# locuoco/coulomb_oscillators

Hardware: AMD Instinct MI355X
Metric: particle-steps/sec (+ Gpair-interactions/sec), N=1048576 FMM-3D kd-tree p=6, 1 GPU(s) (higher is better)
Workload: dtype f32; 1 GPU; FMM-3D kd-tree p=6, N=1048576 per GPU (one system of 1048576), leapfrog, Gaussian ball, tree rebuilt every 1 step(s); n_per_gpu=1048576, order=6, parallelism=single GPU, L=15, p2p_pairs=2017200, m2l_pairs=570291, build_mode=0, warm_builds=281, warm_misses=10, near_field=one-directional

## Files before the change

coulomb_oscillators_amd/csrc/k_fmm_kd.hip:

```cpp
#include "nbco_internal.hpp"
#include "k_p2p.hpp"
#include "kd_common.hpp"
#include "host_util.hpp"
#include <chrono>
#include <cmath>
#include <algorithm>
#include <vector>

namespace {

using kdc::wave_scan_add;
using kdc::wave_min_u32;

constexpr int sym_off(int n) { return n * (n + 1) * (n + 2) / 6; }
constexpr int tl_off(int n) { return n * n; }

struct TreeView
{
	float *center, *lbound, *rbound;
	float4 *csz;
	float *mpole, *local;
	int *mult, *index, *splitdim;
	int L, ntot;
};
// ... 50 lines not shown
	__host__ __device__ uint64_t operator()(unsigned cnt) const { return (uint64_t)cnt | ((uint64_t)((cnt + kP2PChunk - 1) / kP2PChunk) << 32); }
};
struct SplitRef
{
	int *s, *o;
	__host__ __device__ SplitRef &operator=(uint64_t v) { *s = (int)(uint32_t)v; *o = (int)(v >> 32); return *this; }
};
struct SplitIter
{
	using iterator_category = std::random_access_iterator_tag;
	using value_type = uint64_t;
	using difference_type = std::ptrdiff_t;
	using pointer = uint64_t *;
	using reference = SplitRef;
	int *s, *o;
	__host__ __device__ SplitRef operator*() const { return SplitRef{s, o}; }
	__host__ __device__ SplitRef operator[](difference_type i) const { return SplitRef{s + i, o + i}; }
	__host__ __device__ SplitIter operator+(difference_type i) const { return SplitIter{s + i, o + i}; }
	__host__ __device__ SplitIter operator-(difference_type i) const { return SplitIter{s - i, o - i}; }
	__host__ __device__ SplitIter &operator+=(difference_type i) { s += i; o += i; return *this; }
	__host__ __device__ SplitIter &operator++() { ++s; ++o; return *this; }
	__host__ __device__ difference_type operator-(const SplitIter &b) const { return s - b.s; }
};
static int build_directed_list(nbco_ctx *c, const int2 *pairs, const int2 *ranks, const int *pref_dev, long long capR, long long npairs_hint, int sub,
                               int self0, int nself, int ntargets, int shift, unsigned *cnt, int *start, uint64_t *keys_tmp, uint64_t *keys_out,
                               DevBuf &scan_tmp, const int *leaf_index = nullptr, const int *leaf_mult = nullptr, int2 *desc = nullptr,
                               int *chunk_off = nullptr, int4 *chunks = nullptr, const MutualLists *mutual = nullptr)
{
	hipStream_t st = c->stream;
	if (desc)
	{
		NBCO_TRY(exclusive_scan(c, scan_tmp, rocprim::make_transform_iterator((const unsigned *)cnt, PackCounts{}), SplitIter{start, chunk_off}, (uint64_t)0,
		                        (size_t)(ntargets + 1)));
	}
	else
		NBCO_TRY(exclusive_scan(c, scan_tmp, (int *)cnt, start, 0, (size_t)(ntargets + 1)));
	hipLaunchKernelGGL(list_fill_kernel, dim3(grid1d(npairs_hint + nself)), dim3(kBlock), 0, st, pairs, ranks, pref_dev, capR, sub, self0, nself, shift,
	                   (const int *)start, keys_tmp, (const int *)chunk_off, ntargets, leaf_index, leaf_mult,
	                   (desc && !mutual) ? chunks : (int4 *)nullptr, mutual ? 1 : 0);
	if (desc)
	{
		MutualLists mu;
		if (mutual) { mu = *mutual; mu.chunk = chunks; mu.chunk_off = chunk_off; mu.self0 = self0; mu.nself = nself; }
		const bool long_kernel = shift >= 11 && shift <= 16 && c->hint_np2p > 0 && 2 * c->hint_np2p > 48LL * (nself > 0 ? nself : ntargets);
		const int long_from = long_kernel ? 512 : 0;
		c->info.long_lists = long_kernel ? 1 : 0;
		hipLaunchKernelGGL(list_segsort_kernel<true>, dim3((ntargets + kBlock / 64 - 1) / (kBlock / 64)), dim3(kBlock), 0, st, (const int *)start, ntargets,
		                   keys_tmp, keys_out, shift, leaf_index, leaf_mult, desc, mu, long_from);
		if (long_kernel)
			hipLaunchKernelGGL(list_longsort_kernel, dim3(256), dim3(kLongBlock), 0, st, (const int *)start,
			                   ntargets, (const uint64_t *)keys_tmp, keys_out, shift, leaf_index, leaf_mult, desc, mu, long_from);
	}
	else
// ... 165 lines not shown
                                                           const unsigned char *__restrict__ have, int *__restrict__ host_word)
{
	const uint64_t mask = (1ull << shift) - 1;
	const int n = *total;
	int missing = 0;
	for (int i = blockIdx.x * kBlock + threadIdx.x; i < n; i += gridDim.x * kBlock)
	{
		const int id = (int)(keys[i] & mask);
		if (!have[id]) missing = id + 1;
	}
	if (missing) { *host_word = missing; __threadfence_system(); }
}
static int launch_let_guard(nbco_ctx *c, const uint64_t *keys, const int *total, int shift, const unsigned char *have, int word, long long hint)
{
	hipLaunchKernelGGL(let_guard_kernel, dim3(grid1d(hint, 2048)), dim3(kBlock), 0, c->stream, keys, total, shift, have,
	                   c->h_flags + kLetWord + 2 * (int)(c->dist.let_epoch & 1) + word);
	NBCO_HIP(hipGetLastError());
	return NBCO_OK;
}

struct KdCounts
{
	long long np2p = 0, nm2l = 0;
	int sel_overflow = 0, react_overflow = 0;
};

static int kd_list_room(nbco_ctx *c, int ntot, long long &capR, long long &cap)
{
	capR = 2 * (((long long)c->o.list_factor * c->list_growth * ntot + 4096 + kTravK - 1) / kTravK);
	cap = capR * kTravK;
	NBCO_TRY(c->reserve(c->frontier_a, sizeof(int2) * (size_t)cap));
	NBCO_TRY(c->reserve(c->frontier_b, sizeof(int2) * (size_t)cap));
	NBCO_TRY(c->reserve(c->p2p_list, sizeof(int2) * 2 * (size_t)cap));
	NBCO_TRY(c->reserve(c->m2l_list, sizeof(int2) * 2 * (size_t)cap));
	NBCO_TRY(c->reserve(c->counters, sizeof(int) * 128));
	c->list_cap = cap;
	return NBCO_OK;
}

static int kd_traverse(nbco_ctx *c, const TreeView &tv, long long n, const Dom dm)
{
	const int L = tv.L, ntot = tv.ntot, nleaf = 1 << L;
	const int self0 = dm.g << (L - dm.d), nself = 1 << (L - dm.d);
	hipStream_t st = c->stream;
	long long capR, cap;
	NBCO_TRY(kd_list_room(c, ntot, capR, cap));
	PhaseScope ph(c, NBCO_PH_TRAVERSE);
	AdmTab tab;
	for (int l = 0; l < 32; ++l)
	{
		long long lo = l <= L ? (n >> l) : 0;
		long long hi = l <= L ? ((n + (1LL << l) - 1) >> l) : 0;
		tab.lo[l] = (int)lo;
		const float e = 1.f / (float)(3 * c->o.fmm_order + 6);
		tab.Mlo[l] = lo > 0 ? std::pow((float)lo / (float)n, e) : 0.f;
		tab.Mhi[l] = hi > 0 ? std::pow((float)hi / (float)n, e) : 0.f;
	}
	int *ctr = c->counters.as<int>();
	int2 *fa = c->frontier_a.as<int2>(), *fb = c->frontier_b.as<int2>();
	const size_t np_ = (size_t)nleaf + 2, nm_ = (size_t)ntot + 2;
	NBCO_TRY(c->reserve(c->list_cnt, sizeof(unsigned) * 2 * (np_ + nm_)));
	unsigned *cnt_p2p = c->list_cnt.as<unsigned>(), *cnt_m2l = cnt_p2p + 2 * np_;
	NBCO_TRY(c->reserve(c->trav_ctr, sizeof(int) * 1024));
	static_assert(kTcInts <= 1024, "traversal counter block");
	int *tctr = c->trav_ctr.as<int>();
	NBCO_TRY(c->flags_begin());
	hipLaunchKernelGGL(traverse_init_kernel, dim3(grid1d((long long)(2 * (np_ + nm_)) / 8 + 1, 256)), dim3(kBlock), 0, st, fa, ctr, 104, tctr,
	                   c->list_cnt.as<unsigned>(), (long long)(2 * (np_ + nm_)), (long long)self0, (long long)(c->o.coll ? nself : 0));
	const int iters = L + NBCO_TRAV_EXTRA;
	for (int it = 0; it < iters; ++it)
	{
		hipLaunchKernelGGL(traverse_kernel, dim3(1024), dim3(kBlock), 0, st, tv, tab, (const int2 *)fa, fb, c->p2p_list.as<int2>(),
		                   c->m2l_list.as<int2>(), c->p2p_list.as<int2>() + cap, c->m2l_list.as<int2>() + cap, ctr, tctr, it, capR,
		                   c->o.tree_radius, c->o.m2l_first, cnt_p2p, cnt_m2l, dm);
		std::swap(fa, fb);
	}
	hipLaunchKernelGGL(traverse_finish_kernel, dim3(1), dim3(1024), 0, st, ctr, tctr, capR, c->list_cnt.as<unsigned>(), (long long)(2 * (np_ + nm_)),
	                   cnt_p2p + self0, c->o.coll ? nself : 0, c->h_flags, iters, ++c->flags_seq);
	NBCO_HIP(hipGetLastError());
	NBCO_HIP(hipEventRecord(c->ev_flags, st));
	return NBCO_OK;
}

static int kd_no_pre_far() { return NBCO_OK; }

template <class PreFar>
static int kd_fields(nbco_ctx *c, const TreeView &tv, const float4 *pos, long long n, int mlt_max, const Dom dm, long long own0, long long own_n,
                     const int *unsort, float *a, const float *param, KdCounts &out, PreFar pre_far, const LetHave *let = nullptr)
{
	const int P = c->o.fmm_order;
	const int L = tv.L, ntot = tv.ntot, nleaf = 1 << L, beg = kd_beg(L);
	const int offL = tl_off(P + 1);
	out = KdCounts{};
	const int self0 = dm.g << (L - dm.d), nself = 1 << (L - dm.d);
	long long capR, cap;
	NBCO_TRY(kd_list_room(c, ntot, capR, cap));
	const int *p2p_pref = c->trav_ctr.as<int>() + kTcP2PPref, *m2l_pref = c->trav_ctr.as<int>() + kTcM2LPref;
	const int shift = L + 1;
	const long long dp2p_cap = c->o.coll ? 2 * cap + nself : 0, dm2l_cap = 2 * cap;
	const long long np2p_hint = c->hint_np2p > 0 ? std::min(cap, c->hint_np2p + c->hint_np2p / 4 + 1024) : cap;
	const long long nm2l_hint = c->hint_nm2l > 0 ? std::min(cap, c->hint_nm2l + c->hint_nm2l / 4 + 1024) : cap;
	const long long dp2p_hint = 2 * np2p_hint + nself;
	const long long max_chunks = c->o.coll ? dp2p_cap / kP2PChunk + nself : 0, chunks_hint = dp2p_hint / kP2PChunk + nself;
	const int mutual_th = (c->o.coll && c->o.p2p_mutual) ? p2p_mutual_halves(mlt_max) : 0;
	const bool mutual = mutual_th > 0;
	c->info.p2p_halves = mutual_th;
	long long react_cap = 0;
	if (mutual)
	{
		if (c->hint_np2p <= 0)
		{
			NBCO_TRY(c->wait_flags());
			c->hint_np2p = c->h_flags[0];
			c->hint_nm2l = c->h_flags[1];
		}
		const long long pairs_room = std::min(cap, c->hint_np2p + c->hint_np2p / 4 + 1024);
		react_cap = 2 * pairs_room + nself;
		NBCO_TRY(c->reserve(c->p2p_react, sizeof(float4) * 32 * (size_t)mutual_th * (size_t)react_cap));
	}
	float4 *near = nullptr;
	auto enqueue_p2p = [&]() -> int {
		NBCO_TRY(c->reserve(c->part, sizeof(float4) * (size_t)max_chunks * (size_t)mlt_max));
		near = c->part.as<float4>();
		PhaseScope ph(c, NBCO_PH_P2P);
		const int4 *pc = c->p2p_chunks.as<int4>();
		const int *pt = c->p2p_chunk_off.as<int>() + nleaf;
		const int2 *pd = c->p2p_desc.as<int2>();
		if (mutual)
		{
			launch_p2p_mutual(c, mutual_th, pos, c->p2p_desc.as<int4>(), pc, pt, chunks_hint, mlt_max, near, c->p2p_react.as<float4>(), react_cap, n);
		}
		else if (mlt_max <= 8) launch_p2p<8>(c, pos, pd, pc, pt, chunks_hint, mlt_max, mlt_max, near, n);
		else if (mlt_max <= 16) launch_p2p<16>(c, pos, pd, pc, pt, chunks_hint, mlt_max, mlt_max, near, n);
		else if (mlt_max <= 32) launch_p2p<32>(c, pos, pd, pc, pt, chunks_hint, mlt_max, mlt_max, near, n);
		else launch_p2p<64>(c, pos, pd, pc, pt, chunks_hint, mlt_max, mlt_max, near, n);
		NBCO_HIP(hipGetLastError());
		static const char *dump_path = std::getenv("NBCO_P2P_DUMP");
		if (dump_path && !mutual) NBCO_TRY(p2p_dump(c, dump_path, pos, pd, pc, pt, c->p2p_start.as<int>() + nleaf, mlt_max, near, n));
		return NBCO_OK;
	};
	{
		NBCO_TRY(c->reserve(c->p2p_keys, sizeof(uint64_t) * (size_t)(dp2p_cap + 1)));
		NBCO_TRY(c->reserve(c->p2p_keys_alt, sizeof(uint64_t) * (size_t)(dp2p_cap + 1)));
		NBCO_TRY(c->reserve(c->m2l_keys, sizeof(uint64_t) * (size_t)(dm2l_cap + 1)));
		NBCO_TRY(c->reserve(c->m2l_keys_alt, sizeof(uint64_t) * (size_t)(dm2l_cap + 1)));
		NBCO_TRY(c->reserve(c->p2p_start, sizeof(int) * (size_t)(nleaf + 2)));
		NBCO_TRY(c->reserve(c->m2l_start, sizeof(int) * (size_t)(ntot + 2)));
		NBCO_TRY(c->fork_mark());
		if (c->o.coll)
		{
			PhaseScope ph(c, NBCO_PH_LISTS);
			unsigned *cp = c->list_cnt.as<unsigned>();
			NBCO_TRY(c->reserve(c->p2p_desc, (mutual ? sizeof(int4) : sizeof(int2)) * (size_t)(dp2p_cap + 1)));
			MutualLists mu;
			if (mutual)
			{
				NBCO_TRY(c->reserve(c->p2p_sec, sizeof(int2) * (size_t)(nleaf + 2)));
				mu.desc4 = c->p2p_desc.as<int4>();
				mu.sec_range = c->p2p_sec.as<int2>();
			}
			NBCO_TRY(c->reserve(c->p2p_chunk_off, sizeof(int) * (size_t)(nleaf + 2)));
			NBCO_TRY(c->reserve(c->p2p_chunks, sizeof(int4) * (size_t)max_chunks));
			NBCO_TRY(build_directed_list(c, c->p2p_list.as<int2>(), c->p2p_list.as<int2>() + cap, p2p_pref, capR, np2p_hint, beg, self0, nself, nleaf, shift, cp,
			                             c->p2p_start.as<int>(), c->p2p_keys.as<uint64_t>(), c->p2p_keys_alt.as<uint64_t>(), c->sort_tmp,
			                             tv.index + beg, tv.mult + beg, c->p2p_desc.as<int2>(), c->p2p_chunk_off.as<int>(), c->p2p_chunks.as<int4>(),
			                             mutual ? &mu : nullptr));
			if (mutual) launch_p2p_link(c, c->p2p_desc.as<int4>(), c->p2p_keys_alt.as<uint64_t>(), c->p2p_start.as<int>(), c->p2p_start.as<int>() + nleaf, shift, dp2p_hint);
			if (let) NBCO_TRY(launch_let_guard(c, c->p2p_keys_alt.as<uint64_t>(), c->p2p_start.as<int>() + nleaf, shift, let->leaf, 1, dp2p_hint));
			c->pc_mult = tv.mult + beg; c->pc_shift = shift; c->pc_total = c->p2p_start.as<int>() + nleaf;
		}
		if (c->o.coll) NBCO_TRY(enqueue_p2p());
		const int f64 = c->o.far_fp64 ? 1 : 0;
		NBCO_HIP(hipMemsetAsync(tv.local, 0, (f64 ? sizeof(double) : sizeof(float)) * (size_t)ntot * offL, c->aux));
		NBCO_TRY(c->fork_wait());
		{
			StreamScope on_aux(c, c->aux);
			NBCO_TRY(pre_far());
			unsigned *cm = c->list_cnt.as<unsigned>() + 2 * ((size_t)nleaf + 2);
			NBCO_TRY(build_directed_list(c, c->m2l_list.as<int2>(), c->m2l_list.as<int2>() + cap, m2l_pref, capR, nm2l_hint, 0, 0, 0, ntot, shift, cm,
			                             c->m2l_start.as<int>(), c->m2l_keys.as<uint64_t>(), c->m2l_keys_alt.as<uint64_t>(), c->scan_tmp_aux));
			if (let) NBCO_TRY(launch_let_guard(c, c->m2l_keys_alt.as<uint64_t>(), c->m2l_start.as<int>() + ntot, shift, let->node, 0, 2 * nm2l_hint));
			{
				PhaseScope ph(c, NBCO_PH_M2L);
				if (f64) NBCO_TRY(launch_m2l_lanes_f64(c, P, tv.csz, (const double *)tv.mpole, (double *)tv.local, c->m2l_keys_alt.as<uint64_t>(), c->m2l_start.as<int>(), shift, ntot));
				else NBCO_TRY(launch_m2l_lanes(c, P, tv.csz, tv.mpole, tv.local, c->m2l_keys_alt.as<uint64_t>(), c->m2l_start.as<int>(), shift, ntot));
			}
			{
				PhaseScope ph(c, NBCO_PH_L2L);
				NBCO_TRY(launch_downward_gen(c, P, tv.center, tv.local, L, dm.d, dm.g, f64));
			}
		}
		NBCO_HIP(hipGetLastError());
	}
	NBCO_TRY(c->join_aux());
	{
		PhaseScope ph(c, NBCO_PH_L2P);
		NBCO_TRY(launch_l2p_gen(c, P, pos, tv.center, tv.local, near, c->p2p_chunk_off.as<int>(), tv.index, mlt_max, unsort, c->o.unsort ? 1 : 0,
		                        param, a, c->o.coll ? 1 : 0, n, L, own0, own_n, mutual ? c->p2p_sec.as<int2>() : nullptr,
		                        mutual ? c->p2p_react.as<float4>() : nullptr, react_cap, 32 * mutual_th, c->o.far_fp64 ? 1 : 0));
	}
	{
		const auto t0 = std::chrono::steady_clock::now();
		NBCO_TRY(c->wait_flags());
		c->host_wait_s += std::chrono::duration<double>(std::chrono::steady_clock::now() - t0).count();
	}
	const int *h = c->h_flags;
	if (h[3] != 0)
	{
		out.sel_overflow = 1;
		return NBCO_OK;
	}
	if (h[2] == 2) return c->fail(NBCO_ERR_HIP, "internal error: the dual tree traversal did not finish in its launches");
	if (h[2] != 0) return c->fail(NBCO_ERR_CAPACITY, "dual tree traversal exceeded the list capacity (raise opts.list_factor or set opts.list_grow)");
	out.np2p = h[0]; out.nm2l = h[1];
	c->hint_np2p = h[0]; c->hint_nm2l = h[1];
	{
		nbco_ctx::LastEval &le = c->last_eval;
		le.valid = true;
		le.center = tv.center; le.csz = tv.csz; le.mpole = tv.mpole; le.mult = tv.mult; le.index = tv.index;
		le.L = L; le.ntot = ntot; le.order = P; le.shift = shift; le.real_bytes = c->o.far_fp64 ? 8 : 4;
		le.pos = pos; le.n = n; le.own0 = own0; le.own_n = own_n;
		le.have_p2p = c->o.coll != 0;
		le.local = tv.local; le.unsort = unsort; le.scatter = c->o.unsort != 0; le.sharded = tv.center != c->kd.center;
	}
	if (mutual && 2LL * h[0] + nself > react_cap) out.react_overflow = 1;
	return NBCO_OK;
}

static int kd_finish_order(nbco_ctx *c, float *p, long long n, KdStepLink *link)
{
	PhaseScope ph(c, NBCO_PH_FINISH);
	hipStream_t st = c->stream;
	NBCO_TRY(c->reserve(c->tmp3, sizeof(float) * 3 * (size_t)n));
	const int *order_in = nullptr;
	int *order_out = nullptr;
// ... 78 lines not shown
	case 6: launch_kd_psi<6>(c, c0, slot, param, psi_dev); break;
	case 7: launch_kd_psi<7>(c, c0, slot, param, psi_dev); break;
	case 8: launch_kd_psi<8>(c, c0, slot, param, psi_dev); break;
	case 9: launch_kd_psi<9>(c, c0, slot, param, psi_dev); break;
	default: launch_kd_psi<10>(c, c0, slot, param, psi_dev); break;
	}
	hipLaunchKernelGGL(kd_slot_sum_kernel, dim3(1), dim3(kBlock), 0, c->stream, (const double *)slot, nleaf, out);
	NBCO_HIP(hipGetLastError());
	NBCO_HIP(hipMemcpyAsync(half_psi_sum, out, sizeof(double), hipMemcpyDeviceToHost, c->stream));
	NBCO_HIP(hipStreamSynchronize(c->stream));
	return NBCO_OK;
}

static bool kd_wants_room(nbco_ctx *c, int rc, const KdCounts &cnt, int ntot)
{
	if (rc == NBCO_ERR_CAPACITY) return c->grow_lists(ntot);
	return rc == NBCO_OK && cnt.react_overflow && !cnt.sel_overflow;
}

static int kd_retry(nbco_ctx *c, int rc, const KdCounts &cnt, bool rebuild, int ntot, bool &again)
{
	again = true;
	if (kd_wants_room(c, rc, cnt, ntot)) return NBCO_OK;
	if (rc != NBCO_OK) return rc;
	if (cnt.sel_overflow)
		return c->demote_build() ? NBCO_OK : c->fail(NBCO_ERR_UNSUPPORTED, "kd-tree build: tie flag raised by the sorting build");
	if (rebuild && c->sel_warm_used) c->note_warm_ok();
	again = false;
	return NBCO_OK;
}

static void kd_commit(nbco_ctx *c, const KdTreeDev &k, long long n, const KdCounts &cnt, bool rebuilt)
{
	c->tree_valid = true;
	c->tree_n = n;
	c->tree_order = k.order;
	c->eval_counter += 1;
	nbco_kd_info &info = c->info;
	info.L = k.L; info.ntot = k.ntot; info.order = k.order; info.mlt_max = k.mlt_max; info.n = k.n;
	info.p2p_pairs = cnt.np2p; info.m2l_pairs = cnt.nm2l; info.rebuilt = rebuilt ? 1 : 0;
	info.directed_p2p = -1;
}

int kd_finish_pending_order(nbco_ctx *c, float *p, long long n, KdStepLink *link)
{
	if (!link->order_pending) return NBCO_OK;
// ... 32 lines not shown
	else hipLaunchKernelGGL(kd_turnaround_kernel<false>, dim3(kPrepGrid), dim3(kPrepBlock), 0, st, NBCO_TURN_ARGS);
#undef NBCO_TURN_ARGS
	NBCO_HIP(hipGetLastError());
	link->prep_done = next_rebuild ? 1 : 2;
	c->order_n = -1;
	c->last_eval.valid = false;
	link->v_now = v_out == v ? nullptr : v_out;
	return NBCO_OK;
}

int fmm_kdtree_eval(nbco_ctx *c, float *p, float *a, long long n, const float *param, KdStepLink *link)
{
	if (n <= 0) return c->fail(NBCO_ERR_ARG, "nbco_fmm_kdtree: n must be positive");
	if (n > 0x7fffffffLL / 4) return c->fail(NBCO_ERR_UNSUPPORTED, "nbco_fmm_kdtree: n too large for 32-bit tree indices");
	const int L = kd_levels(n, c->o.fmm_order, c->o.dens_inhom, c->o.tree_L);
	const Dom whole{0, 0};
	bool rebuild = false;
	KdCounts cnt;
	for (bool again = true; again;)
	{
		NBCO_TRY(kd_build(c, p, n, L, KdRoot{}, rebuild, link));
		NBCO_TRY(kd_upward(c));
		const TreeView tv = view_of(c->kd);
		int rc = kd_traverse(c, tv, n, whole);
		if (rc == NBCO_OK) rc = kd_fields(c, tv, c->pos4.as<float4>(), n, c->kd.mlt_max, whole, 0, n, c->unsort.as<int>(), a, param, cnt, kd_no_pre_far);
		NBCO_TRY(kd_retry(c, rc, cnt, rebuild, c->kd.ntot, again));
	}
	if (!c->o.unsort && rebuild)
	{
		if (link && link->defer_order) link->order_pending = true;
		else NBCO_TRY(kd_finish_order(c, p, n, link));
	}
	kd_commit(c, c->kd, n, cnt, rebuild);
	return NBCO_OK;
}

#include "kd_dist.hpp"
#include "kd_let.hpp"
int kd_count_pairs(nbco_ctx *c, long long *out)
{
	if (!c->pc_mult || !c->p2p_keys_alt.ptr) { *out = 0; return NBCO_OK; }
	unsigned long long *ctr = (unsigned long long *)(c->counters.as<int>() + 100);
	NBCO_HIP(hipMemsetAsync(ctr, 0, sizeof(unsigned long long), c->stream));
	hipLaunchKernelGGL(pair_count_kernel, dim3(1024), dim3(kBlock), 0, c->stream, c->pc_mult, (const uint64_t *)c->p2p_keys_alt.as<uint64_t>(), c->pc_total,
	                   c->pc_shift, ctr);
	NBCO_HIP(hipGetLastError());
	unsigned long long v = 0;
// ... 49 lines not shown
```

coulomb_oscillators_amd/csrc/kd_list_kernels.hpp:

```cpp

__global__ __launch_bounds__(kBlock) void list_fill_kernel(const int2 *__restrict__ pairs, const int2 *__restrict__ ranks, const int *__restrict__ pref,
                                                           long long capR, int sub, int self0, int nself, int shift, const int *__restrict__ start,
                                                           uint64_t *__restrict__ keys, const int *__restrict__ chunk_off, int ntargets,
                                                           const int *__restrict__ leaf_index, const int *__restrict__ leaf_mult,
                                                           int4 *__restrict__ chunk, int pidmode)
{
	if (chunk)
		for (int i = blockIdx.x * kBlock + threadIdx.x; i < ntargets; i += gridDim.x * kBlock)
		{
			const int b = start[i], e = start[i + 1], o = chunk_off[i], n = chunk_off[i + 1] - o;
			const int ind = leaf_index[i], mlt = leaf_mult[i];
			const int per = n > 0 ? (e - b + n - 1) / n : 0;
			for (int k = 0; k < n; ++k) chunk[o + k] = make_int4(ind, min(b + k * per, e), min(b + (k + 1) * per, e), mlt);
		}
	const long long npairs = pref[kTravK];
	const long long total = npairs + nself;
	for (long long i = (long long)blockIdx.x * kBlock + threadIdx.x; i < total; i += (long long)gridDim.x * kBlock)
	{
		if (i < npairs)
		{
			const long long slot = region_slot(pref, capR, i);
			if (!NBCO_CHECKED_OK(slot >= 0 && slot < capR * kTravK, NBCO_CHK_FILL)) continue;
			const int2 p = pairs[slot], r = ranks[slot];
			const uint64_t a = (uint64_t)(p.x - sub), b = (uint64_t)(p.y - sub);
// ... 2 lines not shown
			if (pidmode)
			{
				if (r.x >= 0) keys[start[a] + r.x] = (b << 32) | (uint64_t)(uint32_t)i;
				if (r.y >= 0) keys[start[b] + r.y] = (a << 32) | (uint64_t)(uint32_t)i;
			}
			else
			{
				if (r.x >= 0) keys[start[a] + r.x] = (a << shift) | b;
				if (r.y >= 0) keys[start[b] + r.y] = (b << shift) | a;
			}
		}
		else
		{
			const uint64_t t = (uint64_t)(self0 + (i - npairs));
			keys[start[t]] = pidmode ? ((t << 32) | 0xFFFFFFFFull) : ((t << shift) | t);
		}
	}
}

#ifndef NBCO_P2P_CHUNK
#define NBCO_P2P_CHUNK 16
#endif
constexpr int kP2PChunk = NBCO_P2P_CHUNK;

static int p2p_dump(nbco_ctx *c, const char *path, const float4 *pos, const int2 *desc, const int4 *chunk, const int *nchunks, const int *nentries, int mlt_max,
                    const float4 *partial, long long n)
{
	NBCO_HIP(hipStreamSynchronize(c->stream));
	int hc = 0, he = 0;
	NBCO_HIP(hipMemcpy(&hc, nchunks, sizeof(int), hipMemcpyDeviceToHost));
	NBCO_HIP(hipMemcpy(&he, nentries, sizeof(int), hipMemcpyDeviceToHost));
	FILE *f = std::fopen(path, "wb");
	if (!f) return c->fail(NBCO_ERR_ARG, "NBCO_P2P_DUMP: cannot open the file");
	const long long head[8] = {n, he, hc, mlt_max, mlt_max, 0, 0, 0};
	std::fwrite(head, sizeof head, 1, f);
	auto put = [&](const void *dev, size_t bytes) {
		std::vector<char> h(bytes);
		if (hipMemcpy(h.data(), dev, bytes, hipMemcpyDeviceToHost) != hipSuccess) return false;
		return std::fwrite(h.data(), 1, bytes, f) == bytes;
	};
	const bool ok = put(pos, sizeof(float4) * (size_t)n) && put(desc, sizeof(int2) * (size_t)he) && put(chunk, sizeof(int4) * (size_t)hc) &&
	                put(partial, sizeof(float4) * (size_t)hc * (size_t)mlt_max);
	std::fclose(f);
	return ok ? NBCO_OK : c->fail(NBCO_ERR_HIP, "NBCO_P2P_DUMP: copy failed");
}
struct MutualLists
// ... 299 lines not shown
```

coulomb_oscillators_amd/csrc/kd_traverse_kernels.hpp:

```cpp

__device__ inline uint64_t block_exclusive_scan3(uint64_t v, uint64_t *sh_wave, uint64_t &total)
{
	const int lane = threadIdx.x & 63, w = threadIdx.x >> 6;
	const uint64_t incl = (uint64_t)wave_scan_add((uint32_t)(v & 0xFFFFFu)) | ((uint64_t)wave_scan_add((uint32_t)((v >> 20) & 0xFFFFFu)) << 20) |
	                      ((uint64_t)wave_scan_add((uint32_t)(v >> 40)) << 40);
	if (lane == 63) sh_wave[w] = incl;
	__syncthreads();
	uint64_t base = 0, tot = 0;
	for (int k = 0; k < 4; ++k)
	{
		uint64_t s = sh_wave[k];
		if (k < w) base += s;
		tot += s;
	}
	total = tot;
	return base + incl - v;
}

__device__ inline int classify_pair(const TreeView &t, const AdmTab *tab, int2 np, float par, int m2l_first, const Dom dm)
{
	const int ntot = t.ntot;
	if (dm.d > 0 && !dom_touch(dm, np.x) && !dom_touch(dm, np.y)) return 0;
	const bool leaf1 = 2 * np.x + 1 >= ntot, leaf2 = 2 * np.y + 1 >= ntot;
	if (!m2l_first && leaf1 && leaf2) return (np.x != np.y) ? 1 : 0;
// ... 36 lines not shown
};
__device__ inline PairKids pair_children(int kd, int2 np)
{
	const int x1 = 2 * np.x + 1, x2 = 2 * np.x + 2, y1 = 2 * np.y + 1, y2 = 2 * np.y + 2;
	PairKids k;
	k.a.x = kd == 4 ? np.x : x1;
	k.a.y = kd == 5 ? np.y : (kd == 4 ? y1 : x1);
	k.b.x = kd == 4 ? np.x : (kd == 5 ? x2 : x1);
	k.b.y = kd == 5 ? np.y : (kd == 4 ? y2 : x2);
	k.c.x = x2;
	k.c.y = x2;
	k.n = kd == 3 ? 3 : (kd >= 4 ? 2 : 0);
	return k;
}

constexpr int kTravK = 16;
constexpr int kTcFrontier = 0;
constexpr int kTcP2P = 36 * kTravK;
constexpr int kTcM2L = kTcP2P + kTravK;
constexpr int kTcP2PPref = kTcM2L + kTravK;
constexpr int kTcM2LPref = kTcP2PPref + kTravK + 1;
constexpr int kTcInts = kTcM2LPref + kTravK + 1;
#ifndef NBCO_TRAV_EXTRA
#define NBCO_TRAV_EXTRA 1
#endif

__device__ inline long long region_slot(const int *__restrict__ pref, long long capR, long long i)
{
	int r = 0;
#pragma unroll
	for (int q = 1; q < kTravK; ++q) r += (i >= pref[q]) ? 1 : 0;
	return (long long)r * capR + (i - pref[r]);
}

__global__ __launch_bounds__(kBlock) void traverse_kernel(TreeView t, AdmTab tab_arg, const int2 *__restrict__ fin, int2 *__restrict__ fout,
                                                          int2 *__restrict__ p2p, int2 *__restrict__ m2l, int2 *__restrict__ p2p_rank,
                                                          int2 *__restrict__ m2l_rank, int *__restrict__ counters,
                                                          int *__restrict__ tctr, int it, long long capR, float par, int m2l_first,
                                                          unsigned *__restrict__ cnt_p2p, unsigned *__restrict__ cnt_m2l, const Dom dm)
{
	__shared__ uint64_t sh_wave[4];
	__shared__ int sh_base[3];
	__shared__ int in_pref[kTravK + 1];
	__shared__ AdmTab tab;
#ifdef NBCO_SUBTREE_PROF
	bool first_pass;
#endif
// ... 185 lines not shown
```

coulomb_oscillators_amd/csrc/nbco_api.hip:

```cpp
#include "nbco_internal.hpp"
#include <chrono>
#include <cstdio>
#include <cmath>
#include <new>
#include <random>

int nbco_ctx::reserve(DevBuf &b, size_t bytes)
{
	nbco_ctx *c = this;
	if (bytes <= b.bytes) return NBCO_OK;
	if (b.ptr)
	{
		NBCO_HIP(hipStreamSynchronize(stream));
		NBCO_HIP(hipFree(b.ptr));
		b.ptr = nullptr;
		b.bytes = 0;
	}
	size_t want = bytes + bytes / 8 + 256;
	NBCO_HIP(hipMalloc(&b.ptr, want));
	b.bytes = want;
	if (poison) NBCO_HIP(hipMemsetAsync(b.ptr, 0x7f, want, stream));
	return NBCO_OK;
}

// ... 149 lines not shown
	if (e != hipSuccess || ndev <= 0)
	{
		fprintf(stderr, "nbco_create: no usable HIP device (%s)\n", e != hipSuccess ? hipGetErrorString(e) : "device count is 0");
		delete c;
		return NBCO_ERR_HIP;
	}
	if (hipGetDevice(&c->device) != hipSuccess) { delete c; return NBCO_ERR_HIP; }
	hipDeviceProp_t prop;
	if (hipGetDeviceProperties(&prop, c->device) == hipSuccess) c->num_cu = prop.multiProcessorCount;
	c->stream = (hipStream_t)c->o.stream;
	c->poison = getenv("NBCO_POISON") && atoi(getenv("NBCO_POISON")) != 0;
	if (getenv("NBCO_SEL_WARM")) c->sel_warm_enabled = atoi(getenv("NBCO_SEL_WARM")) != 0;
	if (hipMalloc(&c->small.ptr, 4096) != hipSuccess) { delete c; return NBCO_ERR_HIP; }
	c->small.bytes = 4096;
	*out = c;
	return NBCO_OK;
}

int nbco_destroy(nbco_ctx *c)
{
	if (c && getenv("NBCO_HOST_TIMING") && c->host_calls)
		fprintf(stderr, "[nbco] nbco_integrate: %lld calls, %.1f us host time per call, of which %.1f us waiting for the traversal flags\n", c->host_calls,
		        1e6 * c->host_call_s / c->host_calls, 1e6 * c->host_wait_s / c->host_calls);
	if (!c) return NBCO_OK;
	if (c->energy_child) { nbco_destroy(c->energy_child); c->energy_child = nullptr; }
	hipStreamSynchronize(c->stream);
	if (c->aux && !c->aux_is_main) { hipStreamSynchronize(c->aux); hipStreamDestroy(c->aux); }
	if (c->ev_fork) hipEventDestroy(c->ev_fork);
	if (c->ev_join) hipEventDestroy(c->ev_join);
	if (c->ev_flags) hipEventDestroy(c->ev_flags);
	if (c->h_flags) hipHostFree(c->h_flags);
	for (auto &t : c->timers)
		for (auto &ev : t.pending) { hipEventDestroy(ev.first); hipEventDestroy(ev.second); }
	delete c;
	return NBCO_OK;
}

int nbco_set_opts(nbco_ctx *c, const nbco_opts *o)
{
	if (!c || !o) return NBCO_ERR_ARG;
	NBCO_TRY(check_opts(c, o));
	if ((hipStream_t)o->stream != c->stream) NBCO_HIP(hipStreamSynchronize(c->stream));
	if (o->list_factor != c->o.list_factor) c->list_growth = 1;
	bool topo = o->fmm_order != c->o.fmm_order || o->dens_inhom != c->o.dens_inhom || o->tree_L != c->o.tree_L
	            || o->unsort != c->o.unsort || o->p2p_mutual != c->o.p2p_mutual || o->track_order != c->o.track_order
	            || o->tree_steps != c->o.tree_steps;
// ... 476 lines not shown
	return NBCO_OK;
}

int nbco_kd_get_info(nbco_ctx *c, nbco_kd_info *info)
{
	if (!c || !info) return NBCO_ERR_ARG;
	if (c->info.directed_p2p < 0 && c->counters.ptr && c->tree_valid)
	{
		long long v = 0;
		NBCO_TRY(kd_count_pairs(c, &v));
		c->info.directed_p2p = v;
	}
	*info = c->info;
	info->build_mode = c->force_sort_build ? 2 : (c->sel_three_pass ? 1 : 0);
	info->warm_builds = c->sel_warm_builds; info->warm_misses = c->sel_warm_misses;
	info->real_bytes = c->kd.real_bytes;
	return NBCO_OK;
}
int nbco_kd_copy(nbco_ctx *c, int which, void *host_dst, long long host_bytes)
{
	if (!c || !host_dst) return NBCO_ERR_ARG;
	return kd_copy_out(c, which, host_dst, host_bytes);
}

int nbco_debug_violations(nbco_ctx *c, long long *out8)
{
	if (!c || !out8) return c ? c->fail(NBCO_ERR_ARG, "nbco_debug_violations: null pointer") : NBCO_ERR_ARG;
	for (int i = 0; i < NBCO_CHK_SITES; ++i) out8[i] = 0;
#ifdef NBCO_CHECKED
	NBCO_HIP(hipDeviceSynchronize());
	unsigned v[NBCO_CHK_SITES] = {};
	NBCO_TRY(nbco_checked_collect_kd(v));
	NBCO_TRY(nbco_checked_collect_oct(v));
	NBCO_TRY(nbco_checked_collect_far(v));
	for (int i = 0; i < NBCO_CHK_SITES; ++i) out8[i] = v[i];
	return NBCO_OK;
#else
	return c->fail(NBCO_ERR_UNSUPPORTED, "nbco_debug_violations: this is not the checked build (libnbco_hip_checked.so)");
#endif
}

int nbco_profile_enable(nbco_ctx *c, int on)
{
	if (!c) return NBCO_ERR_ARG;
	c->profiling = on < 0 ? 0xFFFFFFFFu : (unsigned)on;
	return NBCO_OK;
// ... 148 lines not shown
```

coulomb_oscillators_amd/csrc/nbco_internal.hpp:

```cpp
#pragma once
#include <hip/hip_runtime.h>
#include <cstdint>
#include <cstdio>
#include <cstring>
#include <string>
#include <utility>
#include <vector>
#include "../../include/nbco.h"

#define NBCO_HIP(call)                                                                           \
	do {                                                                                         \
		hipError_t e_ = (call);                                                                  \
		if (e_ != hipSuccess) return c->fail_hip(e_, #call, __FILE__, __LINE__);                 \
	} while (0)

#define NBCO_HIP_M(ctx_, call)                                                                   \
	do {                                                                                         \
		hipError_t e_ = (call);                                                                  \
		if (e_ != hipSuccess) return (ctx_)->fail_hip(e_, #call, __FILE__, __LINE__);            \
	} while (0)

#define NBCO_TRY(call)                   \
	do {                                 \
		int rc_ = (call);                \
// ... 87 lines not shown
{
	nbco_opts o;
	hipStream_t stream = nullptr;
	hipStream_t aux = nullptr;
	hipEvent_t ev_fork = nullptr, ev_join = nullptr;
	bool aux_pending = false;
	int list_growth = 1;
	bool grow_lists(int ntot)
	{
		if (!o.list_grow || list_growth >= 64) return false;
		if (8LL * list_growth * o.list_factor * (long long)ntot + 16384 + ntot >= (1LL << 31)) return false;
		list_growth *= 2;
		return true;
	}
	long long perm_primed_n = -1;
	double host_wait_s = 0, host_call_s = 0;
	long long host_calls = 0;
	bool aux_is_main = false;
	bool poison = false;
	int *h_flags = nullptr;
	hipEvent_t ev_flags = nullptr;
	long long hint_np2p = 0, hint_nm2l = 0;
	int flags_begin();
	int flags_seq = 0;
	int wait_flags();
	DevBuf scan_tmp_aux;
	int fork_aux();
	int fork_mark();
	int fork_wait();
	int join_aux();
	std::string err;
	int device = 0;
	int num_cu = 256;

	DevBuf pos4;
	DevBuf pos4_alt;
	DevBuf part;
	DevBuf small;
	DevBuf tmp3, tmp3b;
	DevBuf keys, keys_alt, idx, idx_alt, unsort, unsort_alt, sort_tmp;
	DevBuf treebuf;
	KdTreeDev kd;
	DevBuf frontier_a, frontier_b, p2p_list, m2l_list, counters;
	DevBuf p2p_keys, p2p_keys_alt, m2l_keys, m2l_keys_alt, p2p_start, m2l_start;
	DevBuf p2p_chunk_off, p2p_chunks, p2p_desc;
	DevBuf order, order_alt;
// ... 190 lines not shown
```

include/nbco.h:

```cpp
#ifndef NBCO_H
#define NBCO_H

#ifdef __cplusplus
extern "C" {
#endif

typedef struct nbco_ctx nbco_ctx;

enum {
	NBCO_OK = 0,
	NBCO_ERR_HIP = 1,
	NBCO_ERR_ARG = 2,
	NBCO_ERR_CAPACITY = 3,
	NBCO_ERR_UNSUPPORTED = 4
};

enum {
	NBCO_EVAL_DIRECT = 0,
	NBCO_EVAL_DIRECT_KAHAN = 1,
	NBCO_EVAL_FMM_KDTREE = 2,
	NBCO_EVAL_FMM_TRACELESS = 3,
	NBCO_EVAL_FMM_SYMMETRIC = 4
};

// ... 156 lines not shown
int nbco_dist_let_local_mpole(nbco_ctx *c, float *buf_local, long long n_local);
int nbco_dist_let_select(nbco_ctx *c, const void *csz_all, long long *counts_send);
int nbco_dist_let_pack(nbco_ctx *c, const long long *counts_all, void *pos_send, void *mpole_send);
int nbco_dist_let_finish(nbco_ctx *c, const long long *counts_all, const void *pos_recv, const void *mpole_recv, float *buf_local,
                         float *a_local, const float *param);
int nbco_dist_let_check(nbco_ctx *c);
int nbco_dist_let_pack_capped(nbco_ctx *c, const long long *caps_out, void *pos_send, void *mpole_send);
int nbco_dist_let_finish_capped(nbco_ctx *c, const long long *caps_in, const void *pos_recv, const void *mpole_recv, float *buf_local,
                                float *a_local, const float *param);
int nbco_dist_let_settle(nbco_ctx *c, int ok);
int nbco_dist_turnaround(nbco_ctx *c, float *buf_local, long long n_local, const float *param, double dt, double scale, int elastic);
int nbco_aux_stream(nbco_ctx *c, void **stream_out);

enum {
	NBCO_PH_BUILD = 0, NBCO_PH_P2M_M2M = 1, NBCO_PH_TRAVERSE = 2, NBCO_PH_LISTS = 3, NBCO_PH_P2P = 4,
	NBCO_PH_M2L = 5, NBCO_PH_L2L = 6, NBCO_PH_L2P = 7, NBCO_PH_FINISH = 8, NBCO_PH_DIRECT = 9,
	NBCO_PH_AXPY = 10, NBCO_PH_COUNT = 11
};
int nbco_profile_enable(nbco_ctx *c, int mask);
int nbco_profile_reset(nbco_ctx *c);
int nbco_profile_get(nbco_ctx *c, int phase, double *total_ms, long long *launches);

int nbco_debug_violations(nbco_ctx *c, long long *out8);

#define NBCO_REF_SEED 5351550349027530206ULL
#define NBCO_REF_DISCARD 1248ULL
int nbco_init_gaussian(float *host_state, long long n, const float *sigma_x3, const float *sigma_u3,
                       unsigned long long seed, unsigned long long discard, int uniform_positions);
int nbco_init_gaussian_slice(float *host_slice, long long n, long long first, long long count, const float *sigma_x3,
                             const float *sigma_u3, unsigned long long seed, unsigned long long discard, int uniform_positions);

enum { NBCO_2D_EVAL_DIRECT = 0, NBCO_2D_EVAL_DIRECT_KAHAN = 1, NBCO_2D_EVAL_FMM = 2 };
int nbco_2d_direct(nbco_ctx *c, const double *p, double *a, long long n, const double *param);
int nbco_2d_direct3(nbco_ctx *c, const double *p, double *a, long long n, const double *param);
int nbco_2d_fmm(nbco_ctx *c, double *p, double *a, long long n, const double *param);
int nbco_2d_force(nbco_ctx *c, int kind, double *buf, long long n, const double *param, int elastic);
int nbco_2d_integrate(nbco_ctx *c, int scheme, int kind, double *buf, long long n, const double *param, double dt, double scale,
                      int elastic);
int nbco_2d_integrate_steps(nbco_ctx *c, int scheme, int kind, double *buf, long long n, const double *param, double dt,
                            double scale, int elastic, int steps);
int nbco_2d_mean_relerr(nbco_ctx *c, const double *x, const double *ref, long long n, double *out_host);
int nbco_2d_energy(nbco_ctx *c, const double *buf, long long n, const double *param, double *out3_host, double *phi_dev);
int nbco_2d_energy_fmm(nbco_ctx *c, const double *buf, long long n, const double *param, double *out3_host, double *phi_dev);
int nbco_2d_probe(nbco_ctx *c, const double *p, long long n, const double *t, long long m, const double *param, double *a_dev,
                  double *psi_dev);
int nbco_2d_probe_fmm(nbco_ctx *c, const double *p, long long n, const double *t, long long m, const double *param, double *a_dev,
// ... 11 lines not shown
```

Before: 674.9 million particle-steps/s.

## Fuse traversal finish into one-launch list offset scans and drop extra traversal pass

Replaces the rocprim exclusive scans that build list offsets with a single custom kernel that computes offsets (and P2P chunk offsets) in one launch. The traversal finish work (prefix of region counters, overflow rule, host flag report) moves into that kernel, which removes a separate finish launch. The default extra traversal iteration is also dropped. If the traversal turns out to be unfinished, the evaluation is retried with more launches. This cuts kernel launches and scan passes on the critical path, but each tile redundantly re-reads all preceding counts and an unfinished traversal now forces a full repeat.

```diff
diff --git a/coulomb_oscillators_amd/csrc/k_fmm_kd.hip b/coulomb_oscillators_amd/csrc/k_fmm_kd.hip
--- a/coulomb_oscillators_amd/csrc/k_fmm_kd.hip
+++ b/coulomb_oscillators_amd/csrc/k_fmm_kd.hip
@@ -96,13 +96,24 @@
 	__host__ __device__ SplitIter &operator++() { ++s; ++o; return *this; }
 	__host__ __device__ difference_type operator-(const SplitIter &b) const { return s - b.s; }
 };
+static bool list_offsets_in_one_launch(int ntargets, const unsigned *cnt)
+{
+	return ntargets + 1 <= kOffMaxCounts && ((uintptr_t)cnt & 15) == 0;
+}
 static int build_directed_list(nbco_ctx *c, const int2 *pairs, const int2 *ranks, const int *pref_dev, long long capR, long long npairs_hint, int sub,
                                int self0, int nself, int ntargets, int shift, unsigned *cnt, int *start, uint64_t *keys_tmp, uint64_t *keys_out,
-                               DevBuf &scan_tmp, const int *leaf_index = nullptr, const int *leaf_mult = nullptr, int2 *desc = nullptr,
+                               DevBuf &scan_tmp, const OffFinish &fin, const int *leaf_index = nullptr, const int *leaf_mult = nullptr, int2 *desc = nullptr,
                                int *chunk_off = nullptr, int4 *chunks = nullptr, const MutualLists *mutual = nullptr)
 {
 	hipStream_t st = c->stream;
-	if (desc)
+	if (list_offsets_in_one_launch(ntargets, cnt))
+	{
+		const int count = ntargets + 1, grid = (count + kOffTile - 1) / kOffTile;
+		if (desc) hipLaunchKernelGGL(list_offsets_kernel<true>, dim3(grid), dim3(kBlock), 0, st, cnt, count, start, chunk_off, self0, nself, fin);
+		else hipLaunchKernelGGL(list_offsets_kernel<false>, dim3(grid), dim3(kBlock), 0, st, cnt, count, start, (int *)nullptr, 0, 0, fin);
+	}
+	else if (fin.mode != 0) return c->fail(NBCO_ERR_HIP, "internal error: fused traversal finish without the one-launch list offsets");
+	else if (desc)
 	{
 		NBCO_TRY(exclusive_scan(c, scan_tmp, rocprim::make_transform_iterator((const unsigned *)cnt, PackCounts{}), SplitIter{start, chunk_off}, (uint64_t)0,
 		                        (size_t)(ntargets + 1)));
@@ -314,7 +325,7 @@
 struct KdCounts
 {
 	long long np2p = 0, nm2l = 0;
-	int sel_overflow = 0, react_overflow = 0;
+	int sel_overflow = 0, react_overflow = 0, trav_left = 0;
 };
 
 static int kd_list_room(nbco_ctx *c, int ntot, long long &capR, long long &cap)
@@ -330,7 +341,13 @@
 	return NBCO_OK;
 }
 
-static int kd_traverse(nbco_ctx *c, const TreeView &tv, long long n, const Dom dm)
+static bool kd_finish_fusable(nbco_ctx *c, int ntot)
+{
+	const unsigned *cp = c->list_cnt.as<unsigned>(), *cm = cp + 2 * ((size_t)(ntot + 1) / 2 + 2);
+	return list_offsets_in_one_launch(ntot, cm) && list_offsets_in_one_launch((ntot + 1) / 2, cp);
+}
+
+static int kd_traverse(nbco_ctx *c, const TreeView &tv, long long n, const Dom dm, bool fuse_finish = false)
 {
 	const int L = tv.L, ntot = tv.ntot, nleaf = 1 << L;
 	const int self0 = dm.g << (L - dm.d), nself = 1 << (L - dm.d);
@@ -359,7 +376,8 @@
 	NBCO_TRY(c->flags_begin());
 	hipLaunchKernelGGL(traverse_init_kernel, dim3(grid1d((long long)(2 * (np_ + nm_)) / 8 + 1, 256)), dim3(kBlock), 0, st, fa, ctr, 104, tctr,
 	                   c->list_cnt.as<unsigned>(), (long long)(2 * (np_ + nm_)), (long long)self0, (long long)(c->o.coll ? nself : 0));
-	const int iters = L + NBCO_TRAV_EXTRA;
+	const int iters = std::max(1, L) + NBCO_TRAV_EXTRA + c->trav_extra;
+	if (iters + 1 > 36) return c->fail(NBCO_ERR_HIP, "internal error: the dual tree traversal needs more launches than its counter block holds");
 	for (int it = 0; it < iters; ++it)
 	{
 		hipLaunchKernelGGL(traverse_kernel, dim3(1024), dim3(kBlock), 0, st, tv, tab, (const int2 *)fa, fb, c->p2p_list.as<int2>(),
@@ -367,8 +385,12 @@
 		                   c->o.tree_radius, c->o.m2l_first, cnt_p2p, cnt_m2l, dm);
 		std::swap(fa, fb);
 	}
+	c->trav_iters = iters;
+	++c->flags_seq;
+	c->finish_fused = fuse_finish && kd_finish_fusable(c, ntot);
+	if (c->finish_fused) { NBCO_HIP(hipGetLastError()); return NBCO_OK; }
 	hipLaunchKernelGGL(traverse_finish_kernel, dim3(1), dim3(1024), 0, st, ctr, tctr, capR, c->list_cnt.as<unsigned>(), (long long)(2 * (np_ + nm_)),
-	                   cnt_p2p + self0, c->o.coll ? nself : 0, c->h_flags, iters, ++c->flags_seq);
+	                   cnt_p2p + self0, c->o.coll ? nself : 0, c->h_flags, iters, c->flags_seq);
 	NBCO_HIP(hipGetLastError());
 	NBCO_HIP(hipEventRecord(c->ev_flags, st));
 	return NBCO_OK;
@@ -402,6 +424,7 @@
 	{
 		if (c->hint_np2p <= 0)
 		{
+			if (c->finish_fused) return c->fail(NBCO_ERR_HIP, "internal error: the flags of a traversal with a fused finish are wanted ahead of its lists");
 			NBCO_TRY(c->wait_flags());
 			c->hint_np2p = c->h_flags[0];
 			c->hint_nm2l = c->h_flags[1];
@@ -439,6 +462,15 @@
 		NBCO_TRY(c->reserve(c->p2p_start, sizeof(int) * (size_t)(nleaf + 2)));
 		NBCO_TRY(c->reserve(c->m2l_start, sizeof(int) * (size_t)(ntot + 2)));
 		NBCO_TRY(c->fork_mark());
+		OffFinish fin_p2p, fin_m2l;
+		if (c->finish_fused)
+		{
+			fin_p2p.mode = kOffRule;
+			fin_m2l.mode = kOffRule | kOffReport | (c->o.coll ? 0 : kOffBoth);
+			fin_p2p.counters = fin_m2l.counters = c->counters.as<int>();
+			fin_p2p.tctr = fin_m2l.tctr = c->trav_ctr.as<int>();
+			fin_m2l.host_flags = c->h_flags; fin_m2l.iters = c->trav_iters; fin_m2l.seq = c->flags_seq;
+		}
 		if (c->o.coll)
 		{
 			PhaseScope ph(c, NBCO_PH_LISTS);
@@ -454,7 +486,7 @@
 			NBCO_TRY(c->reserve(c->p2p_chunk_off, sizeof(int) * (size_t)(nleaf + 2)));
 			NBCO_TRY(c->reserve(c->p2p_chunks, sizeof(int4) * (size_t)max_chunks));
 			NBCO_TRY(build_directed_list(c, c->p2p_list.as<int2>(), c->p2p_list.as<int2>() + cap, p2p_pref, capR, np2p_hint, beg, self0, nself, nleaf, shift, cp,
-			                             c->p2p_start.as<int>(), c->p2p_keys.as<uint64_t>(), c->p2p_keys_alt.as<uint64_t>(), c->sort_tmp,
+			                             c->p2p_start.as<int>(), c->p2p_keys.as<uint64_t>(), c->p2p_keys_alt.as<uint64_t>(), c->sort_tmp, fin_p2p,
 			                             tv.index + beg, tv.mult + beg, c->p2p_desc.as<int2>(), c->p2p_chunk_off.as<int>(), c->p2p_chunks.as<int4>(),
 			                             mutual ? &mu : nullptr));
 			if (mutual) launch_p2p_link(c, c->p2p_desc.as<int4>(), c->p2p_keys_alt.as<uint64_t>(), c->p2p_start.as<int>(), c->p2p_start.as<int>() + nleaf, shift, dp2p_hint);
@@ -470,7 +502,8 @@
 			NBCO_TRY(pre_far());
 			unsigned *cm = c->list_cnt.as<unsigned>() + 2 * ((size_t)nleaf + 2);
 			NBCO_TRY(build_directed_list(c, c->m2l_list.as<int2>(), c->m2l_list.as<int2>() + cap, m2l_pref, capR, nm2l_hint, 0, 0, 0, ntot, shift, cm,
-			                             c->m2l_start.as<int>(), c->m2l_keys.as<uint64_t>(), c->m2l_keys_alt.as<uint64_t>(), c->scan_tmp_aux));
+			                             c->m2l_start.as<int>(), c->m2l_keys.as<uint64_t>(), c->m2l_keys_alt.as<uint64_t>(), c->scan_tmp_aux, fin_m2l));
+			if (c->finish_fused) NBCO_HIP(hipEventRecord(c->ev_flags, c->stream));
 			if (let) NBCO_TRY(launch_let_guard(c, c->m2l_keys_alt.as<uint64_t>(), c->m2l_start.as<int>() + ntot, shift, let->node, 0, 2 * nm2l_hint));
 			{
 				PhaseScope ph(c, NBCO_PH_M2L);
@@ -502,7 +535,11 @@
 		out.sel_overflow = 1;
 		return NBCO_OK;
 	}
-	if (h[2] == 2) return c->fail(NBCO_ERR_HIP, "internal error: the dual tree traversal did not finish in its launches");
+	if (h[2] == 2)
+	{
+		out.trav_left = 1;
+		return c->fail(NBCO_ERR_HIP, "internal error: the dual tree traversal did not finish in its launches");
+	}
 	if (h[2] != 0) return c->fail(NBCO_ERR_CAPACITY, "dual tree traversal exceeded the list capacity (raise opts.list_factor or set opts.list_grow)");
 	out.np2p = h[0]; out.nm2l = h[1];
 	c->hint_np2p = h[0]; c->hint_nm2l = h[1];
@@ -627,6 +664,12 @@
 {
 	again = true;
 	if (kd_wants_room(c, rc, cnt, ntot)) return NBCO_OK;
+	if (cnt.trav_left && c->trav_extra < 4)
+	{
+		++c->trav_extra;
+		++c->trav_repeats;
+		return NBCO_OK;
+	}
 	if (rc != NBCO_OK) return rc;
 	if (cnt.sel_overflow)
 		return c->demote_build() ? NBCO_OK : c->fail(NBCO_ERR_UNSUPPORTED, "kd-tree build: tie flag raised by the sorting build");
@@ -705,7 +748,8 @@
 		NBCO_TRY(kd_build(c, p, n, L, KdRoot{}, rebuild, link));
 		NBCO_TRY(kd_upward(c));
 		const TreeView tv = view_of(c->kd);
-		int rc = kd_traverse(c, tv, n, whole);
+		const bool early_look = c->o.coll && c->o.p2p_mutual && c->hint_np2p <= 0;
+		int rc = kd_traverse(c, tv, n, whole, !early_look);
 		if (rc == NBCO_OK) rc = kd_fields(c, tv, c->pos4.as<float4>(), n, c->kd.mlt_max, whole, 0, n, c->unsort.as<int>(), a, param, cnt, kd_no_pre_far);
 		NBCO_TRY(kd_retry(c, rc, cnt, rebuild, c->kd.ntot, again));
 	}
diff --git a/coulomb_oscillators_amd/csrc/kd_list_kernels.hpp b/coulomb_oscillators_amd/csrc/kd_list_kernels.hpp
--- a/coulomb_oscillators_amd/csrc/kd_list_kernels.hpp
+++ b/coulomb_oscillators_amd/csrc/kd_list_kernels.hpp
@@ -48,6 +48,105 @@
 #define NBCO_P2P_CHUNK 16
 #endif
 constexpr int kP2PChunk = NBCO_P2P_CHUNK;
+
+constexpr int kOffTile = 4 * kBlock;
+constexpr int kOffMaxCounts = 1 << 16;
+constexpr int kOffRule = 1, kOffReport = 2, kOffBoth = 4;
+struct OffFinish
+{
+	int mode = 0;
+	int *counters = nullptr, *tctr = nullptr, *host_flags = nullptr;
+	int iters = 0, seq = 0;
+};
+template <bool P2P>
+__global__ __launch_bounds__(kBlock) void list_offsets_kernel(unsigned *cnt, int count, int *__restrict__ start, int *__restrict__ chunk_off, int self0,
+                                                              int nself, const OffFinish fin)
+{
+	__shared__ uint32_t sh_pre[2][kBlock / 64], sh_tile[2][kBlock / 64];
+	const int lane = threadIdx.x & 63, w = threadIdx.x >> 6;
+	const int tile0 = blockIdx.x * kOffTile;
+	const bool ovf = fin.mode != 0 && fin.counters[2] != 0;
+	auto chunks_of = [](uint32_t v) { return (v + kP2PChunk - 1) / kP2PChunk; };
+	auto ruled = [&](int i) { return (P2P && i >= self0 && i < self0 + nself) ? 1u : 0u; };
+	uint32_t pe = 0, pc = 0;
+	const uint4 *c4 = reinterpret_cast<const uint4 *>(cnt);
+	if (!ovf)
+	{
+#pragma unroll 8
+		for (int j = threadIdx.x; j < tile0 / 4; j += kBlock)
+		{
+			const uint4 v = c4[j];
+			pe += v.x + v.y + v.z + v.w;
+			if (P2P) pc += chunks_of(v.x) + chunks_of(v.y) + chunks_of(v.z) + chunks_of(v.w);
+		}
+	}
+	else if (P2P && threadIdx.x == 0) pe = pc = (uint32_t)max(0, min(tile0, self0 + nself) - self0);
+	const int i0 = tile0 + 4 * (int)threadIdx.x;
+	uint32_t e[4] = {0u, 0u, 0u, 0u};
+	if (i0 < count)
+	{
+		const uint4 v = ovf ? make_uint4(ruled(i0), ruled(i0 + 1), ruled(i0 + 2), ruled(i0 + 3)) : c4[i0 / 4];
+		e[0] = v.x; e[1] = i0 + 1 < count ? v.y : 0u; e[2] = i0 + 2 < count ? v.z : 0u; e[3] = i0 + 3 < count ? v.w : 0u;
+	}
+	const uint32_t te = e[0] + e[1] + e[2] + e[3];
+	const uint32_t tc = P2P ? chunks_of(e[0]) + chunks_of(e[1]) + chunks_of(e[2]) + chunks_of(e[3]) : 0u;
+	const uint32_t ie = wave_scan_add(te), ic = P2P ? wave_scan_add(tc) : 0u;
+	pe = wave_scan_add(pe);
+	if (P2P) pc = wave_scan_add(pc);
+	if (lane == 63) { sh_pre[0][w] = pe; sh_pre[1][w] = pc; sh_tile[0][w] = ie; sh_tile[1][w] = ic; }
+	__syncthreads();
+	uint32_t be = 0, bc = 0;
+#pragma unroll
+	for (int k = 0; k < kBlock / 64; ++k)
+	{
+		be += sh_pre[0][k] + (k < w ? sh_tile[0][k] : 0u);
+		bc += sh_pre[1][k] + (k < w ? sh_tile[1][k] : 0u);
+	}
+	be += ie - te; bc += ic - tc;
+	if (i0 + 3 < count)
+	{
+		*reinterpret_cast<int4 *>(start + i0) = make_int4((int)be, (int)(be + e[0]), (int)(be + e[0] + e[1]), (int)(be + e[0] + e[1] + e[2]));
+		if (P2P)
+			*reinterpret_cast<int4 *>(chunk_off + i0) = make_int4((int)bc, (int)(bc + chunks_of(e[0])), (int)(bc + chunks_of(e[0]) + chunks_of(e[1])),
+			                                                      (int)(bc + chunks_of(e[0]) + chunks_of(e[1]) + chunks_of(e[2])));
+		if (ovf) *reinterpret_cast<uint4 *>(cnt + i0) = make_uint4(e[0], e[1], e[2], e[3]);
+	}
+	else
+	{
+#pragma unroll
+		for (int k = 0; k < 4; ++k)
+		{
+			if (i0 + k < count)
+			{
+				start[i0 + k] = (int)be;
+				if (P2P) chunk_off[i0 + k] = (int)bc;
+				if (ovf) cnt[i0 + k] = e[k];
+			}
+			be += e[k]; bc += chunks_of(e[k]);
+		}
+	}
+	if (fin.mode == 0 || blockIdx.x != 0 || threadIdx.x >= 64) return;
+	int total[2] = {0, 0};
+	for (int which = 0; which < 2; ++which)
+	{
+		const int src = which ? kTcM2L : kTcP2P, dst = which ? kTcM2LPref : kTcP2PPref;
+		const int v = (lane < kTravK && !ovf) ? fin.tctr[src + lane] : 0, incl = (int)wave_scan_add((uint32_t)v);
+		total[which] = __builtin_amdgcn_readlane(incl, kTravK - 1);
+		if (which != (P2P ? 0 : 1) && !(fin.mode & kOffBoth)) continue;
+		if (lane < kTravK) fin.tctr[dst + lane] = incl - v;
+		if (lane == kTravK - 1) { fin.tctr[dst + kTravK] = incl; fin.counters[which] = incl; }
+	}
+	if (!(fin.mode & kOffReport)) return;
+	int left = lane < kTravK ? fin.tctr[kTcFrontier + fin.iters * kTravK + lane] : 0;
+	for (int o = 32; o > 0; o >>= 1) left += __shfl_xor(left, o);
+	if (lane == 0)
+	{
+		fin.host_flags[0] = total[0]; fin.host_flags[1] = total[1];
+		fin.host_flags[2] = ovf ? 1 : (left != 0 ? 2 : 0); fin.host_flags[3] = fin.counters[110];
+	}
+	__threadfence_system();
+	if (lane == 0) __hip_atomic_store(&fin.host_flags[4], fin.seq, __ATOMIC_RELEASE, __HIP_MEMORY_SCOPE_SYSTEM);
+}
 
 static int p2p_dump(nbco_ctx *c, const char *path, const float4 *pos, const int2 *desc, const int4 *chunk, const int *nchunks, const int *nentries, int mlt_max,
                     const float4 *partial, long long n)
diff --git a/coulomb_oscillators_amd/csrc/kd_traverse_kernels.hpp b/coulomb_oscillators_amd/csrc/kd_traverse_kernels.hpp
--- a/coulomb_oscillators_amd/csrc/kd_traverse_kernels.hpp
+++ b/coulomb_oscillators_amd/csrc/kd_traverse_kernels.hpp
@@ -82,7 +82,7 @@
 constexpr int kTcM2LPref = kTcP2PPref + kTravK + 1;
 constexpr int kTcInts = kTcM2LPref + kTravK + 1;
 #ifndef NBCO_TRAV_EXTRA
-#define NBCO_TRAV_EXTRA 1
+#define NBCO_TRAV_EXTRA 0
 #endif
 
 __device__ inline long long region_slot(const int *__restrict__ pref, long long capR, long long i)
diff --git a/coulomb_oscillators_amd/csrc/nbco_api.hip b/coulomb_oscillators_amd/csrc/nbco_api.hip
--- a/coulomb_oscillators_amd/csrc/nbco_api.hip
+++ b/coulomb_oscillators_amd/csrc/nbco_api.hip
@@ -195,6 +195,8 @@
 	if (c && getenv("NBCO_HOST_TIMING") && c->host_calls)
 		fprintf(stderr, "[nbco] nbco_integrate: %lld calls, %.1f us host time per call, of which %.1f us waiting for the traversal flags\n", c->host_calls,
 		        1e6 * c->host_call_s / c->host_calls, 1e6 * c->host_wait_s / c->host_calls);
+	if (c && getenv("NBCO_HOST_TIMING") && c->trav_repeats)
+		fprintf(stderr, "[nbco] %lld evaluations repeated with a longer traversal (now %d launches beyond the tree depth)\n", c->trav_repeats, c->trav_extra);
 	if (!c) return NBCO_OK;
 	if (c->energy_child) { nbco_destroy(c->energy_child); c->energy_child = nullptr; }
 	hipStreamSynchronize(c->stream);
@@ -717,6 +719,8 @@
 	if (!c || !host_dst) return NBCO_ERR_ARG;
 	return kd_copy_out(c, which, host_dst, host_bytes);
 }
+
+long long nbco_debug_trav_repeats(nbco_ctx *c) { return c ? c->trav_repeats : -1; }
 
 int nbco_debug_violations(nbco_ctx *c, long long *out8)
 {
diff --git a/coulomb_oscillators_amd/csrc/nbco_internal.hpp b/coulomb_oscillators_amd/csrc/nbco_internal.hpp
--- a/coulomb_oscillators_amd/csrc/nbco_internal.hpp
+++ b/coulomb_oscillators_amd/csrc/nbco_internal.hpp
@@ -133,6 +133,10 @@
 	hipEvent_t ev_flags = nullptr;
 	long long hint_np2p = 0, hint_nm2l = 0;
 	int flags_begin();
+	bool finish_fused = false;
+	int trav_iters = 0;
+	int trav_extra = 0;
+	long long trav_repeats = 0;
 	int flags_seq = 0;
 	int wait_flags();
 	DevBuf scan_tmp_aux;
diff --git a/include/nbco.h b/include/nbco.h
--- a/include/nbco.h
+++ b/include/nbco.h
@@ -202,6 +202,7 @@
 int nbco_profile_get(nbco_ctx *c, int phase, double *total_ms, long long *launches);
 
 int nbco_debug_violations(nbco_ctx *c, long long *out8);
+long long nbco_debug_trav_repeats(nbco_ctx *c);
 
 #define NBCO_REF_SEED 5351550349027530206ULL
 #define NBCO_REF_DISCARD 1248ULL
```

Result: faster. 682.0 million particle-steps/s, median of 6 (+1.0%).
